# RapidAI/RapidDoc

Hardware: AMD Instinct MI355X
Metric: pages/sec (layout+OCR det/rec) (higher is better)
Workload: dtype f32

## Files before the change

### rapiddoc_amd/csrc/engine.cpp

```cpp
#include "engine.h"

#include <algorithm>
#include <cmath>
#include <cstdio>
#include <cstdlib>
#include <cstring>
#include <sstream>

namespace rd {

namespace {
struct JsonCur {
    const char* p;
    const char* end;
    void ws() {
        while (p < end && (*p == ' ' || *p == '\n' || *p == '\t' || *p == '\r')) ++p;
    }
    bool eat(char c) {
        ws();
        if (p < end && *p == c) { ++p; return true; }
        return false;
    }
    void expect(char c) {
        if (!eat(c)) throw Error(std::string("safetensors header: expected '") + c + "'");
// ... 639 lines not shown
    p.M = x.n * x.h * x.w; p.K = cin; p.Ng = 4 * cout;
    OpRecord r;
    r.name = wname;
    r.kind = "deconv2x2";
    r.cfg = conv_igemm_config_name(p);
    r.flops = 2.0 * p.M * (double)cin * 4 * cout;
    r.bytes = 4.0 * ((double)p.M * cin + (double)p.M * 4 * cout);
    const TView xv = x, yv = y;
    const bool h3 = h3_ && p.wh != nullptr;
    r.run = [p, xv, yv, h3](const Plan& pl, const RunCtx& c) {
        ConvParams q = p;
        q.x = pl.vptr(xv, c);
        q.y = pl.vptr(yv, c);
        if (h3) launch_conv_igemm_h3(q, c.stream);
        else launch_conv_igemm(q, c.stream);
    };
    emit(std::move(r));
    return y;
}

TView Builder::stem3x3s2(const std::string& wname, const std::string& bn, const TView& xin, int act) {
    const HostTensor& w = ws_->get(wname);
    RD_CHECK(w.shape.size() == 4 && w.shape[1] == 3 && w.shape[2] == 3 && w.shape[3] == 3, "stem weight shape");
    const int cout = (int)w.shape[0];
    RD_CHECK(cout % 8 == 0, "stem Cout % 8");
    const int oh = out_dim(xin.h, 3, 2, 1, 1), ow = out_dim(xin.w, 3, 2, 1, 1);
    TView y = alloc(xin.n, oh, ow, cout);
    const std::string key = wname + "|" + bn + "|stem";
    if (!planning()) {
        if (!pb_->has(key + "#w")) {
            std::vector<float> shift;
            std::vector<float> scale = bn_scale_shift(bn, cout, shift);
            std::vector<float> wf((size_t)27 * cout);
            const float* src = w.f32();
            for (int co = 0; co < cout; ++co)
                for (int ci = 0; ci < 3; ++ci)
                    for (int a = 0; a < 3; ++a)
                        for (int b = 0; b < 3; ++b)
                            wf[(size_t)((a * 3 + b) * 3 + ci) * cout + co] = src[(((size_t)co * 3 + ci) * 3 + a) * 3 + b] * scale[co];
            pb_->add(key + "#w", wf);
            pb_->add(key + "#b", shift);
        }
        return y;
    }
    StemParams p{};
    p.N = xin.n; p.H = xin.h; p.W = xin.w; p.in_ch = xin.c;
    p.w = pb_->ptr(key + "#w");
    p.bias = pb_->ptr(key + "#b");
    p.yld = plan_->ld(y);
    p.OH = oh; p.OW = ow; p.Cout = cout;
    p.act = act;
    OpRecord r;
    r.name = wname;
    r.kind = "stem3x3s2";
    r.flops = 2.0 * xin.n * oh * ow * 27.0 * cout;
    r.bytes = 4.0 * ((double)xin.n * xin.c * xin.h * xin.w + (double)xin.n * oh * ow * cout);
    const TView xv = xin, yv = y;
    r.run = [p, xv, yv](const Plan& pl, const RunCtx& c) {
        StemParams q = p;
        q.x = pl.vptr(xv, c);
        q.y = pl.vptr(yv, c);
        launch_stem_conv3x3s2(q, c.stream);
    };
    emit(std::move(r));
    return y;
}

TView Builder::stem_front(const std::string& w1, const std::string& bn1, const std::string& w2a, const std::string& bn2a,
                          const std::string& w2b, const std::string& bn2b, const TView& xin) {
    const int c1 = weight_dim(w1, 0);
    ConvGeom g2;
    g2.kh = g2.kw = 2;
    g2.pb = g2.pr = 1;
    const std::string fkey = w1 + "|" + bn1 + "|stemfront";
    const bool off = std::getenv("RD_STEM_FUSED") && std::getenv("RD_STEM_FUSED")[0] == '0';
    const bool fused = planning() && !off && (h3_ || mixer_h3_) && pb_->has(fkey + "#img");
    if (!fused) {
        TView e = stem3x3s2(w1, bn1, xin, ACT_RELU);
        mask_cols(e, 1);
        TView a = conv(w2a, "", bn2a, e, g2, ACT_RELU);
        mask_cols(a, 1);
        TView cat = alloc(e.n, e.h, e.w, 2 * c1);
        TView cat_pool = slice(cat, 0, c1), cat_b = slice(cat, c1, c1);
        maxpool2x2s1(e, cat_pool);
        conv(w2b, "", bn2b, a, g2, ACT_RELU, &cat_b);
        mask_cols(cat_b, 1);
        release(e);
        release(a);
        if (!planning() && stem_fused_supported(c1) && !pb_->has(fkey + "#img")) {
            const std::string k1 = w1 + "|" + bn1 + "|stem", k2a = w2a + "|" + bn2a, k2b = w2b + "|" + bn2b;
            const float* f1 = pb_->host_ptr(k1 + "#w");
            const float* f2a = pb_->host_ptr(k2a + "#w");
            const float* f2b = pb_->host_ptr(k2b + "#w");
            const int na = c1 / 2;
            const bool fits = fits_fp16_range(std::vector<float>(f1, f1 + (size_t)27 * c1)) &&
                              fits_fp16_range(std::vector<float>(f2a, f2a + (size_t)na * 4 * c1)) &&
                              fits_fp16_range(std::vector<float>(f2b, f2b + (size_t)c1 * 4 * na));
            if (fits && weight_dim(w2a, 0) == na && weight_dim(w2a, 1) == c1 && weight_dim(w2b, 0) == c1 && weight_dim(w2b, 1) == na) {
                std::vector<uint16_t> img;
                prepare_stem_fused_weights(c1, f1, f2a, f2b, img);
                pb_->add_u16(fkey + "#img", img);
                std::vector<float> bias;
                const float* b1 = pb_->host_ptr(k1 + "#b");
                bias.insert(bias.end(), b1, b1 + c1);
                const float* b2a = pb_->host_ptr(k2a + "#b");
                bias.insert(bias.end(), b2a, b2a + na);
                const float* b2b = pb_->host_ptr(k2b + "#b");
                bias.insert(bias.end(), b2b, b2b + c1);
                pb_->add(fkey + "#bias", bias);
            }
        }
        return cat;
    }
    const int oh = out_dim(xin.h, 3, 2, 1, 1), ow = out_dim(xin.w, 3, 2, 1, 1);
    TView cat = alloc(xin.n, oh, ow, 2 * c1);
    const uint16_t* img = reinterpret_cast<const uint16_t*>(pb_->ptr(fkey + "#img"));
    const float* bias = pb_->ptr(fkey + "#bias");
    OpRecord r;
    r.name = w1 + ":front";
    r.kind = "stem_fused";
    r.cfg = "C" + std::to_string(c1);
    r.shape = "N" + std::to_string(xin.n) + "_" + std::to_string(oh) + "x" + std::to_string(ow);
    const int na = c1 / 2;
    r.flops = 2.0 * xin.n * oh * ow * (27.0 * c1 + 4.0 * c1 * na + 4.0 * na * c1);
    r.bytes = 4.0 * ((double)xin.n * xin.c * xin.h * xin.w + (double)xin.n * oh * ow * 2 * c1);
    const TView xv = xin, yv = cat;
    unsigned* flag = range_flag_;
    const bool has_lt = has_lt_;
    const TView ltv = lt_;
    r.run = [xv, yv, img, bias, c1, flag, has_lt, ltv](const Plan& pl, const RunCtx& c) {
        launch_stem_fused(c1, pl.vptr(xv, c), xv.n, xv.h, xv.w, xv.c, img, bias, pl.vptr(yv, c), pl.ld(yv), flag, c.stream,
                          has_lt ? reinterpret_cast<const int32_t*>(pl.vptr(ltv, c)) : nullptr);
    };
    emit(std::move(r));
    return cat;
}

TView Builder::stem_tail(const std::string& w3, const std::string& bn3, const std::string& w4, const std::string& bn4, const TView& x, int act3,
                         int act4, const TView* out, int s3) {
    const int n1 = weight_dim(w3, 0), cin = weight_dim(w3, 1), n2 = weight_dim(w4, 0);
    ConvGeom g3;
    g3.kh = g3.kw = 3;
    g3.sh = g3.sw = s3;
    g3.pt = g3.pl = g3.pb = g3.pr = 1;
    ConvGeom g1;
    if (s3 != 2) {
        TView s3v = conv(w3, "", bn3, x, g3, act3);
        TView s4v = conv(w4, "", bn4, s3v, g1, act4, out);
        release(s3v);
        return s4v;
    }
    const std::string fkey = w3 + "|" + bn3 + "|" + w4 + "|" + bn4 + "|stemtail";
    const int oh = out_dim(x.h, 3, 2, 1, 1), ow = out_dim(x.w, 3, 2, 1, 1);
    const bool fused = planning() && stem34_enabled() && (h3_ || mixer_h3_) && pb_->has(fkey + "#w3") && plan_->ld(x) % 4 == 0 &&
                       (size_t)x.h * x.w * plan_->ld(x) < ((size_t)1 << 30) && (!out || (plan_->ld(*out) % 4 == 0 && out->coff % 4 == 0)) &&
                       (size_t)oh * ow * (out ? plan_->ld(*out) : n2) < ((size_t)1 << 29);
    if (!fused) {
        TView s3 = conv(w3, "", bn3, x, g3, act3);
        TView s4 = conv(w4, "", bn4, s3, g1, act4, out);
        release(s3);
        if (!planning() && stem34_enabled() && !pb_->has(fkey + "#w3") && stem34_shape_ok(cin, n1, n2) && weight_dim(w3, 2) == 3 && weight_dim(w3, 3) == 3 &&
            weight_dim(w4, 1) == n1) {
            const std::string k3 = w3 + "|" + bn3, k4 = w4 + "|" + bn4;
            const float* f3 = pb_->host_ptr(k3 + "#w");
            const float* f4 = pb_->host_ptr(k4 + "#w");
            if (fits_fp16_range(std::vector<float>(f3, f3 + (size_t)n1 * 9 * cin)) && fits_fp16_range(std::vector<float>(f4, f4 + (size_t)n2 * n1))) {
                std::vector<uint16_t> img3, img4;
                float inv[2];
                prepare_stem34_weights(f3, f4, cin, n1, n2, img3, img4, inv);
                pb_->add_u16(fkey + "#w3", img3);
                pb_->add_u16(fkey + "#w4", img4);
                std::vector<float> b3((size_t)((n1 + 31) / 32) * 32, 0.f), b4((size_t)n2, 0.f);
                if (pb_->has(k3 + "#b")) std::copy(pb_->host_ptr(k3 + "#b"), pb_->host_ptr(k3 + "#b") + n1, b3.begin());
                if (pb_->has(k4 + "#b")) std::copy(pb_->host_ptr(k4 + "#b"), pb_->host_ptr(k4 + "#b") + n2, b4.begin());
                pb_->add(fkey + "#b3", b3);
                pb_->add(fkey + "#b4", b4);
                pb_->add(fkey + "#inv", std::vector<float>{inv[0], inv[1]});
            }
        }
        return s4;
    }
    TView y = out ? *out : alloc(x.n, oh, ow, n2);
    RD_CHECK(y.n == x.n && y.h == oh && y.w == ow && y.c == n2, "stem_tail output view mismatch: " + w4);
    Stem34Params p{};
    p.xld = plan_->ld(x);
    p.N = x.n; p.H = x.h; p.W = x.w; p.Cin = cin;
    p.yld = plan_->ld(y);
    p.OH = oh; p.OW = ow; p.N1 = n1; p.N2 = n2;
    p.w3 = reinterpret_cast<const uint16_t*>(pb_->ptr(fkey + "#w3"));
    p.w4 = reinterpret_cast<const uint16_t*>(pb_->ptr(fkey + "#w4"));
    p.b3 = pb_->ptr(fkey + "#b3");
    p.b4 = pb_->ptr(fkey + "#b4");
    p.w3_inv = pb_->host_ptr(fkey + "#inv")[0];
    p.w4_inv = pb_->host_ptr(fkey + "#inv")[1];
    p.act3 = act3; p.act4 = act4;
    p.range_flag = range_flag_;
    OpRecord r;
    r.name = w3 + ":tail";
    r.kind = "stem_tail";
    r.cfg = "C" + std::to_string(cin) + "_" + std::to_string(n1) + "_" + std::to_string(n2);
    r.shape = "M" + std::to_string(x.n * oh * ow) + "_K" + std::to_string(9 * cin) + "_N" + std::to_string(n1) + "_N" + std::to_string(n2);
    r.flops = 2.0 * x.n * oh * ow * (9.0 * cin * n1 + (double)n1 * n2);
    r.bytes = 4.0 * ((double)x.pixels() * cin + (double)x.n * oh * ow * n2 + 9.0 * cin * n1 + (double)n1 * n2);
    const TView xv = x, yv = y;
    r.run = [p, xv, yv](const Plan& pl, const RunCtx& c) mutable {
        Stem34Params q = p;
        q.x = pl.vptr(xv, c);
        q.y = pl.vptr(yv, c);
        launch_stem34(q, c.stream);
    };
    emit(std::move(r));
    return y;
}

TView Builder::seqconv(const std::string& wname, const std::string& bn, const TView& x0, const TView* x1, int act, const TView* tokinfo) {
    const HostTensor& w = ws_->get(wname);
    RD_CHECK(w.shape.size() == 4 && w.shape[3] == 3 && (w.shape[2] == 1 || w.shape[2] == 3), "seqconv weight shape [Cout][Cin][1|3][3]: " + wname);
    const int cout = (int)w.shape[0], cin = (int)w.shape[1], kh = (int)w.shape[2];
    const int c0 = x0.c, c1 = x1 ? x1->c : 0;
    RD_CHECK(cin == c0 + c1, "seqconv Cin mismatch: " + wname);
    const int coutp = (cout + 63) / 64 * 64;
    RD_CHECK(seqconv_shape_ok(c0, c1, coutp), "seqconv: channel counts (segments % 16): " + wname);
    RD_CHECK(x0.h == 1 && (!x1 || (x1->h == 1 && x1->n == x0.n && x1->w == x0.w)), "seqconv: one row of tokens per line: " + wname);
    const bool ragged = tokinfo != nullptr;
    RD_CHECK(!ragged || x0.n == 1, "ragged seqconv: one token row");
    TView yp = alloc(x0.n, 1, x0.w, coutp);
    TView y = coutp == cout ? yp : slice(yp, 0, cout);
    const int K = 3 * cin;
    const std::string key = wname + "|" + bn + "|seq";
    if (!planning()) {
        if (!pb_->has(key + "#w")) {
            std::vector<float> shift;
            std::vector<float> scale = bn_scale_shift(bn, cout, shift);
            std::vector<float> wf((size_t)coutp * K, 0.f);
            shift.resize(coutp, 0.f);
            const float* src = w.f32();
            const int mid = kh / 2;
            for (int co = 0; co < cout; ++co)
                for (int ci = 0; ci < cin; ++ci)
                    for (int t = 0; t < 3; ++t) wf[(size_t)co * K + (size_t)t * cin + ci] = src[(((size_t)co * cin + ci) * kh + mid) * 3 + t] * scale[co];
            pb_->add(key + "#w", wf);
            pb_->add(key + "#b", shift);
            if (fits_fp16_range(wf)) {
                std::vector<uint16_t> hi, lo;
                split_weights_h3(wf.data(), coutp, K, hi, lo);
                pb_->add_u16(key + "#wh", hi);
                pb_->add_u16(key + "#wl", lo);
            }
        }
        return y;
    }
    SeqConvParams p{};
    p.ld0 = plan_->ld(x0); p.C0 = c0;
    p.ld1 = x1 ? plan_->ld(*x1) : 0; p.C1 = c1;
    RD_CHECK(p.ld0 % 4 == 0 && x0.coff % 4 == 0 && p.ld1 % 4 == 0 && (!x1 || x1->coff % 4 == 0), "seqconv: 16-byte aligned token rows");
    p.w = pb_->ptr(key + "#w");
    p.bias = pb_->ptr(key + "#b");
    const bool split = (h3_ || mixer_h3_) && pb_->has(key + "#wh");
    if (split) {
        p.wh = reinterpret_cast<const uint16_t*>(pb_->ptr(key + "#wh"));
        p.wl = reinterpret_cast<const uint16_t*>(pb_->ptr(key + "#wl"));
        p.range_flag = range_flag_;
    }
    p.yld = plan_->ld(yp);
    p.M = (int)x0.pixels(); p.N = coutp;
    p.T = x0.w;
    p.act = act;
    OpRecord r;
    r.name = wname;
    r.kind = "seqconv1x3";
    r.cfg = std::string(c1 ? "2seg" : "1seg") + (ragged ? "/ragged" : "/uniform") + (split ? "/h3" : "/f32");
    r.shape = "M" + std::to_string(p.M) + "_K" + std::to_string(K) + "_N" + std::to_string(cout);
    r.flops = 2.0 * p.M * (double)K * cout;
    r.bytes = 4.0 * ((double)p.M * cin + (double)p.M * cout) + 4.0 * (double)cout * K;
    const TView x0v = x0, x1v = x1 ? *x1 : TView{}, yv = yp, tiv = ragged ? *tokinfo : TView{};
    const bool has1 = x1 != nullptr;
    r.run = [p, x0v, x1v, yv, tiv, has1, ragged](const Plan& pl, const RunCtx& c) {
        SeqConvParams q = p;
        q.x0 = pl.vptr(x0v, c);
        q.x1 = has1 ? pl.vptr(x1v, c) : nullptr;
        q.y = pl.vptr(yv, c);
        q.tokinfo = ragged ? reinterpret_cast<const int32_t*>(pl.vptr(tiv, c)) : nullptr;
        launch_seqconv(q, c.stream);
    };
    emit(std::move(r));
    return y;
}

void Builder::mask_cols(const TView& v, int col) {
    if (!has_lt_ || !planning()) return;
    OpRecord r;
    r.name = "mask_cols";
    r.kind = "mask";
    r.bytes = 4.0 * v.pixels() * v.c;
    const TView yv = v, ltv = lt_;
    r.run = [yv, ltv, col](const Plan& pl, const RunCtx& c) {
        launch_mask_cols(pl.vptr(yv, c), pl.ld(yv), yv.n, yv.h, yv.w, yv.c, reinterpret_cast<const int32_t*>(pl.vptr(ltv, c)) + col,
                         kLineTabStride, c.stream);
    };
    emit(std::move(r));
}

TView Builder::dwconv(const std::string& wname, const std::string& bname, const std::string& bn, const TView& x,
                      const ConvGeom& g, int act, const TView* out, const TView* res, GapOut* gap, const TView* tokinfo) {
    const HostTensor& w = ws_->get(wname);
    RD_CHECK(w.shape.size() == 4 && w.shape[1] == 1, "depthwise weight shape: " + wname);
    const int c = (int)w.shape[0], kh = (int)w.shape[2], kw = (int)w.shape[3];
    RD_CHECK(c == x.c && c % 4 == 0, "depthwise channel mismatch: " + wname);
    RD_CHECK(kh == g.kh && kw == g.kw, "depthwise kernel mismatch: " + wname);
    const int oh = out_dim(x.h, kh, g.sh, g.pt, g.pb), ow = out_dim(x.w, kw, g.sw, g.pl, g.pr);
    TView y = out ? *out : alloc(x.n, oh, ow, c);
    RD_CHECK(y.h == oh && y.w == ow && y.c == c, "depthwise output view mismatch: " + wname);
    const std::string key = wname + "|" + bn + "|dw";
    if (gap) {
// ... 1309 lines not shown
```

### rapiddoc_amd/csrc/kernels_stem34.hip

```cpp
#include <algorithm>
#include <cmath>
#include <cstdlib>
#include <type_traits>
#include <vector>

#include "rd_device.h"

namespace rd {

static constexpr int S34_WAVES = 4;
static constexpr int S34_SLAB_STEPS = 9;

typedef _Float16 s34_f16x2 __attribute__((ext_vector_type(2)));
__device__ __forceinline__ void s34_split4(const f32x4 v, float neg1, f16x4& hi, f16x4& lo) {
#pragma unroll
    for (int e = 0; e < 4; e += 2) {
        const s34_f16x2 h = __builtin_convertvector(f32x2{v[e], v[e + 1]}, s34_f16x2);
        hi[e] = h[0];
        hi[e + 1] = h[1];
        lo[e] = (_Float16)__builtin_fmaf((float)h[0], neg1, v[e]);
        lo[e + 1] = (_Float16)__builtin_fmaf((float)h[1], neg1, v[e + 1]);
    }
}

template <int TR>
struct S34Geom {
    static constexpr int SEG = S34_WAVES / TR;
    static constexpr int TC = 32 * SEG;
    static constexpr int PH = 2 * TR + 1, PW = 2 * TC + 1;
    static constexpr int NE = TC + 1;
    static constexpr int PP = PH * PW;
    static constexpr int SUB = PP * 16;
    static constexpr int PATCH = 4 * SUB;
    static constexpr int NSLOT = (PP * 8 + 255) / 256;
};

template <int NB>
struct S34Frag { f16x8 xh, xl, wh[NB], wl[NB]; };

template <int NB, int MB, int TR, bool HALF>
__global__ void __launch_bounds__(256, 2) conv3x3s2_pw_h1_kernel(Stem34Params p, int tiles_r, int tiles_c, int ntiles) {
    using G = S34Geom<TR>;
    extern __shared__ __attribute__((aligned(16))) unsigned char smem[];
    constexpr int SLAB = NB * 2 * 1024;
    constexpr int WPASS = S34_SLAB_STEPS * SLAB;
    constexpr int WPIECES = WPASS / 1024;
    constexpr int K2 = 2 * NB - (HALF ? 1 : 0);
    constexpr int NSLOT = G::NSLOT;
    const int tid = threadIdx.x, lane = tid & 63;
    const int wave = __builtin_amdgcn_readfirstlane(tid >> 6);
    const int l31 = lane & 31, lhi = lane >> 5;
    unsigned char* Pt = smem;
    unsigned char* Wb = smem + G::PATCH;
    float* Bs = reinterpret_cast<float*>(Wb + WPASS);
    float neg1 = -1.f;
    asm volatile("" : "+s"(neg1));
    const int passes = p.Cin / 16;

    auto dma_pass = [&](int ps) {
        if (p.abl & 16) return;
        const unsigned char* src = reinterpret_cast<const unsigned char*>(p.w3) + (size_t)ps * WPASS + lane * 16;
        unsigned char* dst = Wb;
#pragma unroll
        for (int u = 0; u < (WPIECES + S34_WAVES - 1) / S34_WAVES; ++u) {
            const int f = wave + u * S34_WAVES;
            if (f < WPIECES)
                __builtin_amdgcn_global_load_lds((const __attribute__((address_space(1))) void*)(src + f * 1024),
                                                 (__attribute__((address_space(3))) void*)(dst + f * 1024), 16, 0, 0);
        }
    };

    unsigned xmax = 0;
    u32x4 pre[NSLOT];
    unsigned pre_ok = 0;
    auto load_patch = [&](int im, int oh0, int ow0, int c0, int halves) {
        if (p.abl & 4) return;
        typedef __amdgpu_buffer_rsrc_t rsrc_t;
        const rsrc_t rx = __builtin_amdgcn_make_buffer_rsrc(const_cast<float*>(p.x + (size_t)im * p.H * p.W * p.xld + c0), 0, 0x7fffffff, 0x00020000);
        int stid = tid;
        asm volatile("" : "+v"(stid));
        pre_ok = 0;
#pragma unroll
        for (int i = 0; i < NSLOT; ++i) {
            const int q = stid + 256 * i;
            const int px = min(q >> 3, G::PP - 1), grp = (q & 7) ^ ((i & 1) << 2);
            const int row = px / G::PW, col = px - row * G::PW;
            const int ih = 2 * oh0 - 1 + row, iw = 2 * ow0 - 1 + col;
            if ((unsigned)ih < (unsigned)p.H && (unsigned)iw < (unsigned)p.W) pre_ok |= 1u << i;
            const unsigned gsel = grp < 4 * halves ? 16u * (unsigned)grp : 0u;
            const unsigned off = ((unsigned)min(max(ih, 0), p.H - 1) * (unsigned)p.W + (unsigned)min(max(iw, 0), p.W - 1)) * (unsigned)p.xld * 4u + gsel;
            pre[i] = __builtin_amdgcn_raw_buffer_load_b128(rx, (int)off, 0, 0);
        }
    };
    auto write_patch = [&](int half) {
        if (p.abl & 2) return;
        int stid = tid;
        asm volatile("" : "+v"(stid));
        const int tsel = ((stid >> 2) & 1) ^ half;
#pragma unroll
        for (int i = 0; i < NSLOT; ++i) {
            const int q = stid + 256 * i;
            if ((i & 1) != tsel || q >= G::PP * 8) continue;
            const int px = q >> 3, grp = q & 3;
            const int row = px / G::PW, col = px - row * G::PW;
            const f32x4 x4 = (pre_ok >> i) & 1u ? __builtin_bit_cast(f32x4, pre[i]) : f32x4{0.f, 0.f, 0.f, 0.f};
            f16x4 hi, lo;
            s34_split4(x4, neg1, hi, lo);
#pragma unroll
            for (int e = 0; e < 4; ++e) xmax = max(xmax, __float_as_uint(x4[e]) & 0x7fffffffu);
            const unsigned pos = (unsigned)(row * G::PW + ((col & 1) ? G::NE + (col >> 1) : (col >> 1)));
            const unsigned o = (unsigned)(grp >> 1) * G::SUB + pos * 16u + (unsigned)(grp & 1) * 8u;
            *reinterpret_cast<f16x4*>(Pt + o) = hi;
            *reinterpret_cast<f16x4*>(Pt + 2 * G::SUB + o) = lo;
        }
    };

    const int wr = wave % TR, wseg = wave / TR;
    const unsigned x_lane = (unsigned)lhi * G::SUB + (unsigned)((2 * wr) * G::PW + 32 * wseg + l31) * 16u;
    const unsigned w_lane = (unsigned)lane * 16u;
    auto read_frag = [&](S34Frag<NB>& f, int tap) {
        const int kh = tap / 3, kw = tap - 3 * kh;
        const unsigned a = x_lane + (unsigned)(kh * G::PW + (kw == 1 ? G::NE : kw == 2 ? 1 : 0)) * 16u;
        f.xh = *reinterpret_cast<const f16x8*>(Pt + a);
        f.xl = *reinterpret_cast<const f16x8*>(Pt + 2 * G::SUB + a);
        const unsigned char* wb = Wb + tap * SLAB + w_lane;
#pragma unroll
        for (int nb = 0; nb < NB; ++nb) {
            f.wh[nb] = *reinterpret_cast<const f16x8*>(wb + (2 * nb) * 1024);
            f.wl[nb] = *reinterpret_cast<const f16x8*>(wb + (2 * nb + 1) * 1024);
        }
    };

    f32x16 acc[NB];
    S34Frag<NB> fr[2];
    auto run_pass = [&]() {
        if (p.abl & 1) return;
        read_frag(fr[0], 0);
#pragma unroll
        for (int s = 0; s < S34_SLAB_STEPS; ++s) {
            S34Frag<NB>& cur = fr[s & 1];
            if (s + 1 < S34_SLAB_STEPS) read_frag(fr[(s + 1) & 1], s + 1);
#pragma unroll
            for (int nb = 0; nb < NB; ++nb) acc[nb] = __builtin_amdgcn_mfma_f32_32x32x16_f16(cur.wh[nb], cur.xh, acc[nb], 0, 0, 0);
#pragma unroll
            for (int nb = 0; nb < NB; ++nb) acc[nb] = __builtin_amdgcn_mfma_f32_32x32x16_f16(cur.wh[nb], cur.xl, acc[nb], 0, 0, 0);
#pragma unroll
            for (int nb = 0; nb < NB; ++nb) acc[nb] = __builtin_amdgcn_mfma_f32_32x32x16_f16(cur.wl[nb], cur.xh, acc[nb], 0, 0, 0);
        }
    };

    auto decode = [&](int v, int& im, int& oh0, int& ow0) {
        const int xcd = v & 7, jj = v >> 3, q = ntiles >> 3, rm = ntiles & 7;
        int t = (xcd < rm ? xcd * (q + 1) : rm * (q + 1) + (xcd - rm) * q) + jj;
        const int tc = t % tiles_c;
        t /= tiles_c;
        const int tr = t % tiles_r;
        im = t / tiles_r;
        oh0 = tr * TR;
        ow0 = tc * G::TC;
    };

    unsigned emax = 0;
    const uint16_t* w4 = p.w4;
    int v = blockIdx.x;
    if (v >= ntiles) return;
    for (int i = tid; i < NB * 32; i += 256) Bs[i] = p.b3[i];
    for (int i = tid; i < MB * 32; i += 256) Bs[NB * 32 + i] = i < p.N2 ? p.b4[i] : 0.f;
    int img, oh0, ow0;
    decode(v, img, oh0, ow0);
    if (p.abl >> 10) {
        const bool late = (p.abl & 512) ? ((int)blockIdx.x >= (int)gridDim.x / 2) : (((int)blockIdx.x >> 3) & 1);
        if (late) for (int i = 0; i < (p.abl >> 10); ++i) __builtin_amdgcn_s_sleep(127);
    }
    dma_pass(0);
    load_patch(img, oh0, ow0, 0, min(2, passes));
    write_patch(0);
    asm volatile("s_waitcnt vmcnt(0) lgkmcnt(0)\n\ts_barrier" ::: "memory");

#pragma unroll 1
    while (true) {
#pragma unroll
        for (int nb = 0; nb < NB; ++nb)
#pragma unroll
            for (int i = 0; i < 16; ++i) acc[nb][i] = 0.f;
        const int vn = v + (int)gridDim.x;
        int img_n = 0, oh_n = 0, ow_n = 0;
        if (vn < ntiles) decode(vn, img_n, oh_n, ow_n);
#pragma unroll 1
        for (int pass = 0; pass < passes; ++pass) {
            const bool last = pass + 1 == passes;
            const bool more = !last || vn < ntiles;
            const bool round_ends = (pass & 1) || last;
            if (round_ends && more) {
                if (!last) load_patch(img, oh0, ow0, (pass + 1) * 16, min(2, passes - pass - 1));
                else load_patch(img_n, oh_n, ow_n, 0, min(2, passes));
            }
            run_pass();
            if (last && !(p.abl & 8)) {
                f16x8 hb[K2], lb[K2];
                int lane_e = lane;
                asm volatile("" : "+v"(lane_e));
                const int lhie = lane_e >> 5, l31e = lane_e & 31;
#pragma unroll
                for (int nb = 0; nb < NB; ++nb) {
#pragma unroll
                    for (int r4 = 0; r4 < 4; ++r4) {
                        if (2 * nb + (r4 >> 1) >= K2) continue;
                        const f32x4 bv = *reinterpret_cast<const f32x4*>(Bs + 32 * nb + 8 * r4 + 4 * lhie);
                        f32x4 h;
#pragma unroll
                        for (int e = 0; e < 4; ++e) {
                            h[e] = fmaf(acc[nb][4 * r4 + e], p.w3_inv, bv[e]);
                            emax = max(emax, __float_as_uint(h[e]) & 0x7fffffffu);
                        }
                        if (p.act3 == ACT_RELU) {
#pragma unroll
                            for (int e = 0; e < 4; ++e) h[e] = fmaxf(h[e], 0.f);
                        } else if (p.act3 != ACT_NONE) {
#pragma unroll
                            for (int e = 0; e < 4; ++e) h[e] = rd_act(h[e], p.act3);
                        }
                        f16x4 hi, lo;
                        s34_split4(h, neg1, hi, lo);
                        const int j = 2 * nb + (r4 >> 1), e0 = 4 * (r4 & 1);
#pragma unroll
                        for (int e = 0; e < 4; ++e) {
                            hb[j][e0 + e] = hi[e];
                            lb[j][e0 + e] = lo[e];
                        }
                    }
                }
                const int oh = oh0 + wr;
                typedef __amdgpu_buffer_rsrc_t rsrc_t;
                const unsigned img_bytes = (unsigned)p.OH * (unsigned)p.OW * (unsigned)p.yld * 4u;
                const rsrc_t ry = __builtin_amdgcn_make_buffer_rsrc(p.y + (size_t)img * p.OH * p.OW * p.yld, 0, (int)img_bytes, 0x00020000);
                const unsigned rowbase = (unsigned)(min(oh, p.OH - 1) * p.OW) * (unsigned)p.yld * 4u;
                const int pw0 = ow0 + 32 * wseg + 4 * lhie;
                unsigned omax = 0;
#pragma unroll
                for (int mb = 0; mb < MB; ++mb) {
                    f32x16 a2;
#pragma unroll
                    for (int i = 0; i < 16; ++i) a2[i] = 0.f;
                    f16x8 wh[K2], wl[K2];
#pragma unroll
                    for (int j = 0; j < K2; ++j) {
                        wh[j] = *reinterpret_cast<const f16x8*>(w4 + ((size_t)(mb * K2 + j) * 2) * 512 + lane_e * 8);
                        wl[j] = *reinterpret_cast<const f16x8*>(w4 + ((size_t)(mb * K2 + j) * 2 + 1) * 512 + lane_e * 8);
                    }
#pragma unroll
                    for (int j = 0; j < K2; ++j) {
                        a2 = __builtin_amdgcn_mfma_f32_32x32x16_f16(hb[j], wh[j], a2, 0, 0, 0);
                        a2 = __builtin_amdgcn_mfma_f32_32x32x16_f16(lb[j], wh[j], a2, 0, 0, 0);
                        a2 = __builtin_amdgcn_mfma_f32_32x32x16_f16(hb[j], wl[j], a2, 0, 0, 0);
                    }
                    const int n = 32 * mb + l31e;
                    const float bv = Bs[NB * 32 + n];
                    const bool nok = n < p.N2 && oh < p.OH && !(p.abl & 32);
                    float o[16];
#pragma unroll
                    for (int i = 0; i < 16; ++i) {
                        o[i] = fmaf(a2[i], p.w4_inv, bv);
                        omax = max(omax, __float_as_uint(o[i]) & 0x7fffffffu);
                    }
                    if (p.act4 == ACT_RELU) {
#pragma unroll
                        for (int i = 0; i < 16; ++i) o[i] = fmaxf(o[i], 0.f);
                    } else if (p.act4 != ACT_NONE) {
#pragma unroll
                        for (int i = 0; i < 16; ++i) o[i] = rd_act(o[i], p.act4);
                    }
#pragma unroll
                    for (int i = 0; i < 16; ++i) {
                        const int pw = pw0 + (i & 3) + 8 * (i >> 2);
                        const unsigned off = (nok && pw < p.OW) ? rowbase + ((unsigned)pw * (unsigned)p.yld + (unsigned)n) * 4u : 0xfffffff0u;
                        __builtin_amdgcn_raw_buffer_store_b32(__float_as_uint(o[i]), ry, (int)off, 0, 2);
                    }
                }
                if (omax >= 0x7f800000u) emax = omax;
            }
            if (!more) break;
            asm volatile("s_barrier" ::: "memory");
            dma_pass(last ? 0 : pass + 1);
            write_patch(last ? 0 : ((pass + 1) & 1));
            asm volatile("s_waitcnt vmcnt(0) lgkmcnt(0)\n\ts_barrier" ::: "memory");
        }
        if (vn >= ntiles) break;
        v = vn; img = img_n; oh0 = oh_n; ow0 = ow_n;
    }
    if ((emax >= 0x477fe000u || xmax >= 0x477fe000u) && p.range_flag) rd_raise_flag(p.range_flag);
}

bool stem34_enabled() {
    static const bool on = [] { const char* e = getenv("RD_STEM34"); return e && e[0] == '1'; }();
    return on;
}
bool stem34_shape_ok(int cin, int n1, int n2) {
    return cin % 16 == 0 && cin >= 16 && cin <= 256 && n1 >= 8 && n1 <= 64 && n1 % 4 == 0 && n2 >= 8 && n2 <= 96 && n2 % 4 == 0 && !(n1 > 48 && n2 > 64);
}

static int wgs_per_cu() {
    static const int n = [] { const char* e = getenv("RD_STEM34_WGS"); return e ? atoi(e) : 2; }();
    return n;
}
template <int NB, int MB, int TR, bool HALF>
static void launch_stem34_t(const Stem34Params& p, hipStream_t s, int n_cu) {
    using G = S34Geom<TR>;
    const int tiles_r = (p.OH + TR - 1) / TR, tiles_c = (p.OW + G::TC - 1) / G::TC;
    const int ntiles = p.N * tiles_r * tiles_c;
    const size_t lds = (size_t)G::PATCH + (size_t)S34_SLAB_STEPS * NB * 2048 + (size_t)(NB + MB) * 32 * sizeof(float);
    static unsigned long long ok = 0;
    rd_allow_dynamic_lds((const void*)conv3x3s2_pw_h1_kernel<NB, MB, TR, HALF>, lds, ok);
    hipLaunchKernelGGL((conv3x3s2_pw_h1_kernel<NB, MB, TR, HALF>), dim3((unsigned)std::min(ntiles, wgs_per_cu() * n_cu)), dim3(256), lds, s, p, tiles_r, tiles_c, ntiles);
}

void launch_stem34(const Stem34Params& p_in, hipStream_t s) {
    if (p_in.N <= 0 || p_in.OH <= 0 || p_in.OW <= 0) return;
    static const int abl = [] { const char* e = getenv("RD_STEM34_ABL"); return e ? atoi(e) : 0; }();
    Stem34Params p = p_in;
    p.abl = abl;
    static const int n_cu = [] {
        int dev = 0, n = 256;
        (void)hipGetDevice(&dev);
        (void)hipDeviceGetAttribute(&n, hipDeviceAttributeMultiprocessorCount, dev);
        return n > 0 ? n : 256;
    }();
    const int nb = (p.N1 + 31) / 32, mb = (p.N2 + 31) / 32;
    auto covered = [&](int tr, int tc) { return (long)((p.OH + tr - 1) / tr * tr) * ((p.OW + tc - 1) / tc * tc); };
    static const int force_tr = [] { const char* e = getenv("RD_STEM34_TR"); return e ? atoi(e) : 0; }();
    const bool tr2 = force_tr ? force_tr == 2 : covered(2, 64) < covered(4, 32);
    const bool half = p.N1 <= 32 * nb - 16;
#define RD_S34_CASE(NBv, MBv, FULL)                                             \
    if (nb == NBv && mb == MBv) {                                               \
        if (half && tr2) launch_stem34_t<NBv, MBv, 2, true>(p, s, n_cu);        \
        else if (half) launch_stem34_t<NBv, MBv, 4, true>(p, s, n_cu);          \
        else if constexpr (FULL) {                                              \
            if (tr2) launch_stem34_t<NBv, MBv, 2, false>(p, s, n_cu);           \
            else launch_stem34_t<NBv, MBv, 4, false>(p, s, n_cu);               \
        }                                                                       \
        return;                                                                 \
    }
    RD_S34_CASE(1, 1, true) RD_S34_CASE(1, 2, true) RD_S34_CASE(1, 3, true) RD_S34_CASE(2, 1, true) RD_S34_CASE(2, 2, true) RD_S34_CASE(2, 3, false)
#undef RD_S34_CASE
}

static float s34_scale_exp(const float* w, size_t n, int& ex) {
    float mx = 0.f;
    for (size_t i = 0; i < n; ++i) mx = std::fmax(mx, std::fabs(w[i]));
    ex = 0;
    if (mx > 0.f && std::isfinite(mx)) {
        int x = 0;
        (void)std::frexp(mx, &x);
        ex = 14 - x;
        ex = ex > 100 ? 100 : ex < -100 ? -100 : ex;
    }
    return std::ldexp(1.f, -ex);
}
static void s34_put(float v, int ex, uint16_t& hb, uint16_t& lb) {
    const float vs = std::ldexp(v, ex);
    const _Float16 hh = (_Float16)vs;
    const _Float16 ll = (_Float16)(vs - (float)hh);
    __builtin_memcpy(&hb, &hh, 2);
    __builtin_memcpy(&lb, &ll, 2);
}

void prepare_stem34_weights(const float* w3, const float* w4, int Cin, int N1, int N2, std::vector<uint16_t>& img3, std::vector<uint16_t>& img4,
                            float inv[2]) {
    const int K = 9 * Cin, nb_n = (N1 + 31) / 32, mb_n = (N2 + 31) / 32, passes = Cin / 16, K2 = 2 * nb_n - (N1 <= 32 * nb_n - 16 ? 1 : 0);
    int ex3 = 0, ex4 = 0;
    inv[0] = s34_scale_exp(w3, (size_t)N1 * K, ex3);
    inv[1] = s34_scale_exp(w4, (size_t)N2 * N1, ex4);
    img3.assign((size_t)passes * 9 * nb_n * 2 * 512, 0);
    size_t slab = 0;
    for (int pass = 0; pass < passes; ++pass)
        for (int tap = 0; tap < 9; ++tap, ++slab)
            for (int nb = 0; nb < nb_n; ++nb)
                for (int lane = 0; lane < 64; ++lane) {
                    const int n = nb * 32 + (lane & 31);
                    if (n >= N1) continue;
                    for (int e = 0; e < 8; ++e) {
                        const int k = tap * Cin + pass * 16 + 8 * (lane >> 5) + e;
                        const size_t base = ((slab * nb_n + nb) * 2) * 512 + (size_t)lane * 8 + e;
                        s34_put(w3[(size_t)n * K + k], ex3, img3[base], img3[base + 512]);
                    }
                }
    img4.assign((size_t)mb_n * K2 * 2 * 512, 0);
    for (int mb = 0; mb < mb_n; ++mb)
        for (int j = 0; j < K2; ++j)
            for (int lane = 0; lane < 64; ++lane) {
                const int n = mb * 32 + (lane & 31);
                if (n >= N2) continue;
                for (int e = 0; e < 8; ++e) {
                    const int c = 16 * j + 8 * (e >> 2) + 4 * (lane >> 5) + (e & 3);
                    if (c >= N1) continue;
                    const size_t base = ((size_t)(mb * K2 + j) * 2) * 512 + (size_t)lane * 8 + e;
                    s34_put(w4[(size_t)n * N1 + c], ex4, img4[base], img4[base + 512]);
                }
            }
}

}
```

### rapiddoc_amd/csrc/rd_kernels.h

```cpp
#pragma once
#include <hip/hip_runtime.h>
#include <cstdint>
#include <cstdlib>
#include <vector>

namespace rd {

inline void rd_allow_dynamic_lds(const void* kernel, size_t bytes, unsigned long long& mask) {
    int dev = 0;
    (void)hipGetDevice(&dev);
    const unsigned long long bit = 1ull << (dev & 63);
    if (!(mask & bit)) {
        (void)hipFuncSetAttribute(kernel, hipFuncAttributeMaxDynamicSharedMemorySize, (int)bytes);
        mask |= bit;
    }
}

inline int rd_cu_budget(int n_cu) {
    static const int env = [] { const char* e = std::getenv("RD_PERSISTENT_CUS"); return e ? std::atoi(e) : 0; }();
    return env > 0 && env < n_cu ? env : n_cu;
}

enum Act : int { ACT_NONE = 0, ACT_RELU = 1, ACT_GELU = 2, ACT_SILU = 3, ACT_SIGMOID = 4, ACT_HSIG = 5, ACT_HSIG_PADDLE = 6 };
enum OutMode : int { OUT_NHWC = 0, OUT_DECONV2X2 = 1 };

struct ConvParams {
    const float* x; int xld;
    int N, H, W, Cin;
    const float* w;
    const uint16_t* wh;
    const uint16_t* wl;
    const float* bias;
    float* y; int yld;
    int OH, OW, Cout;
    int KH, KW, SH, SW, PT, PL;
    const float* res; int rld;
    const float* ascale;
    const float* ln_g; const float* ln_b;
    int act, out_mode;
    int M, K, Ng;
    unsigned* range_flag = nullptr;
    const uint16_t* w1 = nullptr;
    float w1_inv = 0.f;
    int allow_skinny = 0;
    const uint16_t* w3 = nullptr;
    float w3_inv = 0.f;
    const uint16_t* w9 = nullptr;
    float w9_inv = 0.f;
    int fast_epi = 1;
};
void launch_conv_igemm(const ConvParams& p, hipStream_t s);
bool skinny_gemm_applies(int M, int K);
bool gemm_h3_dma_applies(const ConvParams& p);
bool gemm_h3_dma_uses16(const ConvParams& p);
void launch_gemm_h3_dma(const ConvParams& p, hipStream_t s);
bool gemm_h1_shape_ok(int K, int cout);
bool gemm_h1_applies(const ConvParams& p);
void launch_gemm_h1(const ConvParams& p, hipStream_t s);
float prepare_gemm_h1_weights(const float* w, int N, int K, std::vector<uint16_t>& img);
void launch_conv_igemm_h3(const ConvParams& p, hipStream_t s);
void launch_msdeform_attn(const float* value, const int32_t* shapes, const int32_t* start, const float* loc, const float* attn, float* out, int B,
                          int S, int H, int D, int Q, int L, int P, hipStream_t s);
void launch_topk_rows(const float* scores, int rows, int n, int k, float* out_vals, int32_t* out_idx, hipStream_t s);
struct Stem34Params {
    const float* x; int xld;
    int N, H, W, Cin;
    float* y; int yld;
    int OH, OW, N1, N2;
    const uint16_t* w3; float w3_inv; const float* b3;
    const uint16_t* w4; float w4_inv; const float* b4;
    int act3, act4;
    unsigned* range_flag = nullptr;
    int abl = 0;
};
bool stem34_shape_ok(int cin, int n1, int n2);
bool stem34_enabled();
void launch_stem34(const Stem34Params& p, hipStream_t s);
void prepare_stem34_weights(const float* w3, const float* w4, int Cin, int N1, int N2, std::vector<uint16_t>& img3, std::vector<uint16_t>& img4,
                            float inv[2]);
bool conv3x3_h1_shape_ok(int kh, int kw, int cin, int cout);
bool conv3x3_h1_applies(const ConvParams& p);
void launch_conv3x3_h1(const ConvParams& p, hipStream_t s);
float prepare_conv3x3_h1_weights(const float* w, int N, int Cin, std::vector<uint16_t>& img);
bool conv9x9_h1_shape_ok(int kh, int kw, int cin, int cout);
bool conv9x9_h1_applies(const ConvParams& p);
void launch_conv9x9_h1(const ConvParams& p, hipStream_t s);
float prepare_conv9x9_h1_weights(const float* w, int N, int Cin, std::vector<uint16_t>& img);
bool conv_direct_h3_supported(const ConvParams& p);
bool conv_direct_h3_applies(const ConvParams& p);
void launch_conv_direct_h3(const ConvParams& p, hipStream_t s);
bool conv_stream_h3_supported(const ConvParams& p);
bool conv_stream_h3_applies(const ConvParams& p);
void launch_conv_stream_h3(const ConvParams& p, hipStream_t s);
inline bool conv_stream_h3_shape_ok(int kh, int kw, int cin, int cout) {
    return cin % 4 == 0 && cin <= 64 && kh * kw * ((cin + 15) / 16 * 16) <= 256 && cout <= 96;
}
struct SeqConvParams {
    const float* x0; int ld0, C0;
    const float* x1; int ld1, C1;
    const float* w;
    const uint16_t* wh; const uint16_t* wl;
    const float* bias;
    float* y; int yld;
    int M, N;
    int T;
    const int32_t* tokinfo;
    int act;
    unsigned* range_flag;
};
bool seqconv_shape_ok(int C0, int C1, int N);
void launch_seqconv(const SeqConvParams& p, hipStream_t s);
const char* conv_igemm_config_name(const ConvParams& p);

struct StemParams {
    const float* x;
    int N, H, W, in_ch;
    const float* w;
    const float* bias;
    float* y; int yld; int OH, OW, Cout;
    int act;
};
void launch_stem_conv3x3s2(const StemParams& p, hipStream_t s);

bool stem_fused_supported(int c1);
void prepare_stem_fused_weights(int c1, const float* w1_stem_layout, const float* w2a_folded, const float* w2b_folded, std::vector<uint16_t>& img);
void launch_stem_fused(int c1, const float* x, int N, int H, int W, int in_ch, const uint16_t* wimg, const float* bias, float* y, int yld,
                       unsigned* range_flag, hipStream_t s, const int32_t* line_tab = nullptr);

constexpr int kLineTabStride = 4;

struct DwParams {
    const float* x; int xld;
    int N, H, W, C;
    const float* w;
    const float* bias;
    float* y; int yld;
    int OH, OW, KH, KW, SH, SW, PT, PL;
    int act;
    const float* res; int rld;
    float* gap_partial;
    int gap_chunks;
    const int32_t* tokinfo = nullptr;
    const int32_t* line_w = nullptr; int line_w_stride = 0;
    int dbg = 0;
};
void launch_dwconv(const DwParams& p, hipStream_t s);
int dwconv_gap_chunks(const DwParams& p);
bool dwconv_lds_applies(const DwParams& p);
int dwconv_lds_gap_chunks(const DwParams& p);
void launch_dwconv_lds(const DwParams& p, hipStream_t s);
bool dwconv_kxk_lds_applies(const DwParams& p);
void launch_dwconv_kxk_lds(const DwParams& p, hipStream_t s);

struct Lcv3DwParams {
    const float* x; int xld;
    int N, H, W, C;
    const float* w;
    const float* bias;
    float* y; int yld;
    int OH, OW, K, SH, SW;
    int pre_act; float pre_s, pre_b;
    float post_s, post_b;
    const int32_t* line_in; const int32_t* line_out; int line_stride;
    int post_act;
};
bool lcv3_dw_shape_ok(int k, int sh, int sw, int c);
void launch_lcv3_dw(const Lcv3DwParams& p, hipStream_t s);
bool lcv3_dw2d_shape_ok(int k, int sh, int sw, int c);
bool lcv3_dw2d_launch_ok(const Lcv3DwParams& p);
bool launch_lcv3_dw2d(const Lcv3DwParams& p, hipStream_t s);
bool dw5_strip_launch_ok(const Lcv3DwParams& p);
bool launch_dw5_strip(const Lcv3DwParams& p, hipStream_t s);
void launch_mv1e_pool(const float* x, int xld, float* y, int yld, int N, int H, int W, int C, hipStream_t s, const int32_t* line_tab = nullptr);
void launch_lcv3_act(const float* x, int xld, float* y, int yld, long pixels, int C, float s, float b, hipStream_t st);
struct Lcv3BlockParams {
    const float* x; int xld;
    int N, H, W, cin, cout;
    const float* dw_w;
    const float* dw_b;
    const float* pw_w;
    const float* pw_b;
    float* y; int yld;
    int pre_act; float pre_s, pre_b;
    float mid_s, mid_b;
    int out_act; float out_s, out_b;
    const int32_t* line_w; int line_stride;
    int split; unsigned* range_flag;
};
bool lcv3_block_shape_ok(int cin, int cout);
void launch_lcv3_block(const Lcv3BlockParams& p, hipStream_t s);
enum Mbv3Act : int { MBV3_NONE = 0, MBV3_RELU = 1, MBV3_HSWISH = 2 };
struct Mbv3DwParams {
    const float* x; int xld;
    int N, H, W, C;
    const float* w;
    const float* bias;
    float* y; int yld;
    int OH, OW, K, S;
    int pre_act, post_act;
    int max_blocks = 0;
};
bool mbv3_dw_shape_ok(int k, int s, int c);
bool mbv3_dw_launch_ok(const Mbv3DwParams& p);
bool launch_mbv3_dw(const Mbv3DwParams& p, hipStream_t s);
struct Mbv3BlockParams {
    const float* x; int xld;
    int N, H, W, cin, mid, cout;
    const float* we; const float* be;
    const float* wd; const float* bd;
    const float* wl; const float* bl;
    float* y; int yld;
    int OH, OW, K, S;
    int act;
    int in_hswish;
    int shortcut;
};
bool mbv3_block_launch_ok(const Mbv3BlockParams& p);
bool launch_mbv3_block(const Mbv3BlockParams& p, hipStream_t s);
struct Mbv3sDwParams {
    const float* x; int xld;
    int N, H, W, C;
    const float* w;
    const float* bias;
    float* y; int yld;
    int OH, OW, K, SH, SW;
    int pre_act, post_act;
    int max_blocks = 0;
};
bool mbv3s_dw_shape_ok(int k, int sh, int sw, int c);
// ... 210 lines not shown
```

Measured before the change: 377.2.

## Double-buffer stem34 patch prefetch and enable fused stem by default for large inputs

The fused 3x3s2 plus pointwise stem kernel now keeps two register buffers of input patches and prefetches one channel pass ahead, including across tile boundaries. It waits only on older loads (vmcnt(NH)) instead of draining all memory operations each pass. Weight slabs are now moved with buffer loads into LDS, and some ablation hooks are removed. The fused path, previously opt-in through an environment variable, is now on by default for two specific stem shapes above an image size threshold, which raises register pressure and brings a new kernel into the default path.

```diff
diff --git a/rapiddoc_amd/csrc/engine.cpp b/rapiddoc_amd/csrc/engine.cpp
--- a/rapiddoc_amd/csrc/engine.cpp
+++ b/rapiddoc_amd/csrc/engine.cpp
@@ -815,14 +815,14 @@
     }
     const std::string fkey = w3 + "|" + bn3 + "|" + w4 + "|" + bn4 + "|stemtail";
     const int oh = out_dim(x.h, 3, 2, 1, 1), ow = out_dim(x.w, 3, 2, 1, 1);
-    const bool fused = planning() && stem34_enabled() && (h3_ || mixer_h3_) && pb_->has(fkey + "#w3") && plan_->ld(x) % 4 == 0 &&
+    const bool fused = planning() && stem34_enabled(cin, n1, n2, x.h, x.w) && (h3_ || mixer_h3_) && pb_->has(fkey + "#w3") && plan_->ld(x) % 4 == 0 &&
                        (size_t)x.h * x.w * plan_->ld(x) < ((size_t)1 << 30) && (!out || (plan_->ld(*out) % 4 == 0 && out->coff % 4 == 0)) &&
                        (size_t)oh * ow * (out ? plan_->ld(*out) : n2) < ((size_t)1 << 29);
     if (!fused) {
         TView s3 = conv(w3, "", bn3, x, g3, act3);
         TView s4 = conv(w4, "", bn4, s3, g1, act4, out);
         release(s3);
-        if (!planning() && stem34_enabled() && !pb_->has(fkey + "#w3") && stem34_shape_ok(cin, n1, n2) && weight_dim(w3, 2) == 3 && weight_dim(w3, 3) == 3 &&
+        if (!planning() && stem34_wants_weights(cin, n1, n2) && !pb_->has(fkey + "#w3") && stem34_shape_ok(cin, n1, n2) && weight_dim(w3, 2) == 3 && weight_dim(w3, 3) == 3 &&
             weight_dim(w4, 1) == n1) {
             const std::string k3 = w3 + "|" + bn3, k4 = w4 + "|" + bn4;
             const float* f3 = pb_->host_ptr(k3 + "#w");
diff --git a/rapiddoc_amd/csrc/kernels_stem34.hip b/rapiddoc_amd/csrc/kernels_stem34.hip
--- a/rapiddoc_amd/csrc/kernels_stem34.hip
+++ b/rapiddoc_amd/csrc/kernels_stem34.hip
@@ -32,7 +32,7 @@
     static constexpr int PP = PH * PW;
     static constexpr int SUB = PP * 16;
     static constexpr int PATCH = 4 * SUB;
-    static constexpr int NSLOT = (PP * 8 + 255) / 256;
+    static constexpr int NH = (PP * 4 + 255) / 256;
 };
 
 template <int NB>
@@ -46,7 +46,7 @@
     constexpr int WPASS = S34_SLAB_STEPS * SLAB;
     constexpr int WPIECES = WPASS / 1024;
     constexpr int K2 = 2 * NB - (HALF ? 1 : 0);
-    constexpr int NSLOT = G::NSLOT;
+    constexpr int NH = G::NH;
     const int tid = threadIdx.x, lane = tid & 63;
     const int wave = __builtin_amdgcn_readfirstlane(tid >> 6);
     const int l31 = lane & 31, lhi = lane >> 5;
@@ -58,50 +58,65 @@
     const int passes = p.Cin / 16;
 
     auto dma_pass = [&](int ps) {
-        if (p.abl & 16) return;
-        const unsigned char* src = reinterpret_cast<const unsigned char*>(p.w3) + (size_t)ps * WPASS + lane * 16;
-        unsigned char* dst = Wb;
+        typedef __amdgpu_buffer_rsrc_t rsrc_t;
+        const rsrc_t rw = __builtin_amdgcn_make_buffer_rsrc(const_cast<uint16_t*>(p.w3), 0, (p.abl & 16) ? 0 : passes * WPASS, 0x00020000);
 #pragma unroll
         for (int u = 0; u < (WPIECES + S34_WAVES - 1) / S34_WAVES; ++u) {
             const int f = wave + u * S34_WAVES;
             if (f < WPIECES)
-                __builtin_amdgcn_global_load_lds((const __attribute__((address_space(1))) void*)(src + f * 1024),
-                                                 (__attribute__((address_space(3))) void*)(dst + f * 1024), 16, 0, 0);
-        }
+                __builtin_amdgcn_raw_ptr_buffer_load_lds(rw, (__attribute__((address_space(3))) void*)(Wb + f * 1024), 16, lane * 16,
+                                                         ps * WPASS + f * 1024, 0, 0);
+        }
+        asm volatile("" ::: "memory");
+    };
+
+    auto decode = [&](int v, int& im, int& oh0, int& ow0) {
+        const int xcd = v & 7, jj = v >> 3, q = ntiles >> 3, rm = ntiles & 7;
+        int t = (xcd < rm ? xcd * (q + 1) : rm * (q + 1) + (xcd - rm) * q) + jj;
+        const int tc = t % tiles_c;
+        t /= tiles_c;
+        const int tr = t % tiles_r;
+        im = t / tiles_r;
+        oh0 = tr * TR;
+        ow0 = tc * G::TC;
     };
 
     unsigned xmax = 0;
-    u32x4 pre[NSLOT];
-    unsigned pre_ok = 0;
-    auto load_patch = [&](int im, int oh0, int ow0, int c0, int halves) {
-        if (p.abl & 4) return;
+    u32x4 RA[NH], RB[NH];
+    unsigned okA = 0, okB = 0;
+    int fv = blockIdx.x, fimg = 0, foh = 0, fow = 0, fpass = 0;
+    auto fetch = [&](u32x4 (&pre)[NH], unsigned& pre_ok) {
         typedef __amdgpu_buffer_rsrc_t rsrc_t;
-        const rsrc_t rx = __builtin_amdgcn_make_buffer_rsrc(const_cast<float*>(p.x + (size_t)im * p.H * p.W * p.xld + c0), 0, 0x7fffffff, 0x00020000);
+        const rsrc_t rx = __builtin_amdgcn_make_buffer_rsrc(const_cast<float*>(p.x + (size_t)fimg * p.H * p.W * p.xld + 16 * fpass), 0,
+                                                            fv < ntiles && !(p.abl & 4) ? 0x7fffffff : 0, 0x00020000);
         int stid = tid;
         asm volatile("" : "+v"(stid));
         pre_ok = 0;
 #pragma unroll
-        for (int i = 0; i < NSLOT; ++i) {
+        for (int i = 0; i < NH; ++i) {
             const int q = stid + 256 * i;
-            const int px = min(q >> 3, G::PP - 1), grp = (q & 7) ^ ((i & 1) << 2);
+            const int px = min(q >> 2, G::PP - 1), grp = q & 3;
             const int row = px / G::PW, col = px - row * G::PW;
-            const int ih = 2 * oh0 - 1 + row, iw = 2 * ow0 - 1 + col;
+            const int ih = 2 * foh - 1 + row, iw = 2 * fow - 1 + col;
             if ((unsigned)ih < (unsigned)p.H && (unsigned)iw < (unsigned)p.W) pre_ok |= 1u << i;
-            const unsigned gsel = grp < 4 * halves ? 16u * (unsigned)grp : 0u;
-            const unsigned off = ((unsigned)min(max(ih, 0), p.H - 1) * (unsigned)p.W + (unsigned)min(max(iw, 0), p.W - 1)) * (unsigned)p.xld * 4u + gsel;
+            const unsigned off = ((unsigned)min(max(ih, 0), p.H - 1) * (unsigned)p.W + (unsigned)min(max(iw, 0), p.W - 1)) * (unsigned)p.xld * 4u + 16u * (unsigned)grp;
             pre[i] = __builtin_amdgcn_raw_buffer_load_b128(rx, (int)off, 0, 0);
         }
-    };
-    auto write_patch = [&](int half) {
+        if (fv < ntiles && ++fpass == passes) {
+            fpass = 0;
+            fv += (int)gridDim.x;
+            if (fv < ntiles) decode(fv, fimg, foh, fow);
+        }
+    };
+    auto write_patch = [&](u32x4 (&pre)[NH], const unsigned pre_ok) {
         if (p.abl & 2) return;
         int stid = tid;
         asm volatile("" : "+v"(stid));
-        const int tsel = ((stid >> 2) & 1) ^ half;
-#pragma unroll
-        for (int i = 0; i < NSLOT; ++i) {
+#pragma unroll
+        for (int i = 0; i < NH; ++i) {
             const int q = stid + 256 * i;
-            if ((i & 1) != tsel || q >= G::PP * 8) continue;
-            const int px = q >> 3, grp = q & 3;
+            if (i == NH - 1 && q >= G::PP * 4) continue;
+            const int px = q >> 2, grp = q & 3;
             const int row = px / G::PW, col = px - row * G::PW;
             const f32x4 x4 = (pre_ok >> i) & 1u ? __builtin_bit_cast(f32x4, pre[i]) : f32x4{0.f, 0.f, 0.f, 0.f};
             f16x4 hi, lo;
@@ -149,52 +164,34 @@
         }
     };
 
-    auto decode = [&](int v, int& im, int& oh0, int& ow0) {
-        const int xcd = v & 7, jj = v >> 3, q = ntiles >> 3, rm = ntiles & 7;
-        int t = (xcd < rm ? xcd * (q + 1) : rm * (q + 1) + (xcd - rm) * q) + jj;
-        const int tc = t % tiles_c;
-        t /= tiles_c;
-        const int tr = t % tiles_r;
-        im = t / tiles_r;
-        oh0 = tr * TR;
-        ow0 = tc * G::TC;
-    };
-
     unsigned emax = 0;
     const uint16_t* w4 = p.w4;
     int v = blockIdx.x;
     if (v >= ntiles) return;
     for (int i = tid; i < NB * 32; i += 256) Bs[i] = p.b3[i];
     for (int i = tid; i < MB * 32; i += 256) Bs[NB * 32 + i] = i < p.N2 ? p.b4[i] : 0.f;
-    int img, oh0, ow0;
+    int img, oh0, ow0, pass = 0;
     decode(v, img, oh0, ow0);
-    if (p.abl >> 10) {
-        const bool late = (p.abl & 512) ? ((int)blockIdx.x >= (int)gridDim.x / 2) : (((int)blockIdx.x >> 3) & 1);
-        if (late) for (int i = 0; i < (p.abl >> 10); ++i) __builtin_amdgcn_s_sleep(127);
-    }
+    fimg = img; foh = oh0; fow = ow0;
+    auto wait_all_but_newest_request = [&]() {
+        asm volatile("s_waitcnt vmcnt(%0) lgkmcnt(0)\n\ts_barrier" ::"n"(NH) : "memory");
+    };
+    fetch(RA, okA);
+    fetch(RB, okB);
+    write_patch(RA, okA);
     dma_pass(0);
-    load_patch(img, oh0, ow0, 0, min(2, passes));
-    write_patch(0);
-    asm volatile("s_waitcnt vmcnt(0) lgkmcnt(0)\n\ts_barrier" ::: "memory");
-
-#pragma unroll 1
-    while (true) {
-#pragma unroll
-        for (int nb = 0; nb < NB; ++nb)
-#pragma unroll
-            for (int i = 0; i < 16; ++i) acc[nb][i] = 0.f;
-        const int vn = v + (int)gridDim.x;
-        int img_n = 0, oh_n = 0, ow_n = 0;
-        if (vn < ntiles) decode(vn, img_n, oh_n, ow_n);
-#pragma unroll 1
-        for (int pass = 0; pass < passes; ++pass) {
+    fetch(RA, okA);
+    wait_all_but_newest_request();
+#pragma unroll
+    for (int nb = 0; nb < NB; ++nb)
+#pragma unroll
+        for (int i = 0; i < 16; ++i) acc[nb][i] = 0.f;
+
+    auto step = [&](u32x4 (&pre)[NH], unsigned& pre_ok) -> bool {
+        {
             const bool last = pass + 1 == passes;
+            const int vn = v + (int)gridDim.x;
             const bool more = !last || vn < ntiles;
-            const bool round_ends = (pass & 1) || last;
-            if (round_ends && more) {
-                if (!last) load_patch(img, oh0, ow0, (pass + 1) * 16, min(2, passes - pass - 1));
-                else load_patch(img_n, oh_n, ow_n, 0, min(2, passes));
-            }
             run_pass();
             if (last && !(p.abl & 8)) {
                 f16x8 hb[K2], lb[K2];
@@ -237,7 +234,8 @@
                 const unsigned rowbase = (unsigned)(min(oh, p.OH - 1) * p.OW) * (unsigned)p.yld * 4u;
                 const int pw0 = ow0 + 32 * wseg + 4 * lhie;
                 unsigned omax = 0;
-#pragma unroll
+                constexpr int MBU = TR == 2 && NB == 2 ? 1 : MB;
+#pragma unroll MBU
                 for (int mb = 0; mb < MB; ++mb) {
                     f32x16 a2;
 #pragma unroll
@@ -279,22 +277,48 @@
                 }
                 if (omax >= 0x7f800000u) emax = omax;
             }
-            if (!more) break;
+            if (!more) return true;
             asm volatile("s_barrier" ::: "memory");
+            write_patch(pre, pre_ok);
             dma_pass(last ? 0 : pass + 1);
-            write_patch(last ? 0 : ((pass + 1) & 1));
-            asm volatile("s_waitcnt vmcnt(0) lgkmcnt(0)\n\ts_barrier" ::: "memory");
-        }
-        if (vn >= ntiles) break;
-        v = vn; img = img_n; oh0 = oh_n; ow0 = ow_n;
+            fetch(pre, pre_ok);
+            wait_all_but_newest_request();
+            if (last) {
+#pragma unroll
+                for (int nb = 0; nb < NB; ++nb)
+#pragma unroll
+                    for (int i = 0; i < 16; ++i) acc[nb][i] = 0.f;
+                v = vn;
+                decode(v, img, oh0, ow0);
+                pass = 0;
+            } else {
+                ++pass;
+            }
+            return false;
+        }
+    };
+#pragma unroll 1
+    while (true) {
+        if (step(RB, okB)) break;
+        if (step(RA, okA)) break;
     }
     if ((emax >= 0x477fe000u || xmax >= 0x477fe000u) && p.range_flag) rd_raise_flag(p.range_flag);
 }
 
-bool stem34_enabled() {
-    static const bool on = [] { const char* e = getenv("RD_STEM34"); return e && e[0] == '1'; }();
-    return on;
-}
+bool stem34_default(int cin, int n1, int n2, int h, int w) {
+    const long px = (long)h * w;
+    if (cin == 48 && n1 == 24 && n2 == 48) return px >= 480L * 352;
+    if (cin == 64 && n1 == 32 && n2 == 48) return px >= 400L * 400;
+    return false;
+}
+static int stem34_forced() {
+    static const int forced = [] { const char* e = getenv("RD_STEM34"); return e && (e[0] == '0' || e[0] == '1') ? e[0] - '0' : -1; }();
+    return forced;
+}
+bool stem34_enabled(int cin, int n1, int n2, int h, int w) {
+    return stem34_forced() >= 0 ? stem34_forced() == 1 : stem34_default(cin, n1, n2, h, w);
+}
+bool stem34_wants_weights(int cin, int n1, int n2) { return stem34_enabled(cin, n1, n2, 1 << 15, 1 << 15); }
 bool stem34_shape_ok(int cin, int n1, int n2) {
     return cin % 16 == 0 && cin >= 16 && cin <= 256 && n1 >= 8 && n1 <= 64 && n1 % 4 == 0 && n2 >= 8 && n2 <= 96 && n2 % 4 == 0 && !(n1 > 48 && n2 > 64);
 }
diff --git a/rapiddoc_amd/csrc/rd_kernels.h b/rapiddoc_amd/csrc/rd_kernels.h
--- a/rapiddoc_amd/csrc/rd_kernels.h
+++ b/rapiddoc_amd/csrc/rd_kernels.h
@@ -74,7 +74,9 @@
     int abl = 0;
 };
 bool stem34_shape_ok(int cin, int n1, int n2);
-bool stem34_enabled();
+bool stem34_default(int cin, int n1, int n2, int h, int w);
+bool stem34_enabled(int cin, int n1, int n2, int h, int w);
+bool stem34_wants_weights(int cin, int n1, int n2);
 void launch_stem34(const Stem34Params& p, hipStream_t s);
 void prepare_stem34_weights(const float* w3, const float* w4, int Cin, int N1, int N2, std::vector<uint16_t>& img3, std::vector<uint16_t>& img4,
                             float inv[2]);
```

Result: no change. 378.2, median of 2 (+0.3%).
